# bingjeff/trex-gym

Hardware: AMD Instinct MI355X
Metric: env-steps/sec (whole node), trex.urdf 4096 envs per MI355X (higher is better)
Workload: dtype f32

## Files before the change

trex-gym_amd/csrc/device_model.h:

```cpp
#pragma once
#include <stdint.h>

#define TREX_TL 32
#define TREX_MAXD 6
#define TREX_MAXCH 4
#define TREX_CM_WORDS 320
#define TREX_MAXC 13

enum TrexParam {
  TP_DT, TP_SUBSTEPS, TP_ITERATIONS, TP_GRAVITY, TP_MOTOR_KP, TP_MOTOR_KD, TP_MOTOR_MAX_FORCE,
  TP_FLOOR_Z, TP_FRICTION, TP_ERP, TP_CONTACT_ERP, TP_CONTACT_MARGIN, TP_LINK_DAMPING,
  TP_MAX_COORD_VEL, TP_MAX_CONTACTS, TP_WARMSTART, TP_COUNT
};

struct TrexDeviceModel {
  int nb, maxdepth, head_body, nv;
  float prm[16];
  int n_substeps, n_iterations, max_contacts, pad0;
  float inv_dt, motor_max_impulse, pad1, pad2;
  float head_point[4];
  float base_pos0[4], base_quat0[4];
  int parent[TREX_TL], depth[TREX_TL];
  int obs_slot[TREX_TL];
  unsigned tree_pack[TREX_TL], child_pack[TREX_TL];
  int hull_range[TREX_TL][2];
  int pad4[64];
  int child[TREX_MAXCH][TREX_TL];
  unsigned desc_mask[TREX_TL];
  int hull_start[TREX_TL + 1];
  int cm_pack[TREX_TL];
  float axis[3][TREX_TL], jpos[3][TREX_TL], jrot[9][TREX_TL], com[3][TREX_TL], inertia[6][TREX_TL];
  float mass[TREX_TL], lower[TREX_TL], upper[TREX_TL], damp[TREX_TL], q_start[TREX_TL];
  float sphere[4][TREX_TL];
  float box_half[3][TREX_TL];
  int nchunk, pad3[3];
  int chunk_body[TREX_TL], chunk_v0[TREX_TL], chunk_v1[TREX_TL];
  float chunk_c[3][TREX_TL], chunk_h[3][TREX_TL];
  __attribute__((aligned(16))) int chunk_row[TREX_TL][4];
  float chunk_box[TREX_TL][8];
  int anc[TREX_MAXD][TREX_TL];
};
#define TREX_NO_DEPTH 255

#define TREX_BASE_FLAGS 13
#define TREX_BASE_IMPULSE 14
#define TREX_BASE_STEPS 15
#define TREX_MOTORS_BIT 256
#define TREX_BAL_PHASE 0
#define TREX_BAL_FINISHED 1
#define TREX_BAL_COUNTS 16
#define TREX_BAL_BINS 16
#define TREX_BAL_LISTS 48
#define TREX_BAL_WORDS(n) (TREX_BAL_LISTS + 2 * TREX_BAL_BINS * (size_t)(n))

struct TrexBatchArrays {
  float *base, *q, *qd, *mass_scale, *friction;
  int32_t domain;
  int32_t pad0_;
  int32_t *balance;
  int32_t max_episode_steps;
  int32_t pad_;
  float4 *hull;
  int num_links;
  const int *link_body;
  const float *link_tf;
  int num_visuals;
  const int *visual_body;
  const float *visual_tf;
};
#define TREX_WARM_WORDS 64
```

trex-gym_amd/csrc/host_tables.cpp:

```cpp
#include "host_tables.hpp"

#include "../../include/trex_policy.h"

#include <algorithm>
#include <array>
#include <cmath>
#include <cstdint>
#include <cstring>

namespace trex {

size_t row_block_bytes(size_t n, int stride, int width) { return ((n - 1) * (size_t)stride + (size_t)width) * sizeof(float); }

bool ranges_overlap(const void *a, size_t na, const void *b, size_t nb) {
  const uintptr_t p = (uintptr_t)a, q = (uintptr_t)b;
  return p < q + nb && q < p + na;
}

void check_env_offset(const std::string &who, uint32_t env_offset, int n_envs) {
  if ((uint64_t)env_offset + (uint64_t)n_envs > (1ull << 32)) throw Refusal(who + "env_offset + N is beyond 2^32");
}

size_t Layout::take(const char *name, size_t member_bytes, size_t align) {
  const size_t at = (bytes + align - 1) / align * align;
// ... 130 lines not shown
        const int g0 = h.hull_group_start[g], g1 = h.hull_group_start[g + 1];
        if (g1 <= g0) continue;
        int body = -1;
        for (int b = 0; b < h.nb; b++)
          if (h.hull_start[b] <= g0 && g1 <= h.hull_start[b + 1]) body = b;
        if (body < 0) ok = false;
        else units.push_back({body, g0, g1});
      }
    if (!ok || units.size() > TREX_TL) {
      units.clear();
      for (int b = 0; b < h.nb; b++)
        if (h.hull_start[b + 1] > h.hull_start[b]) units.push_back({b, h.hull_start[b], h.hull_start[b + 1]});
    }
    d.nchunk = (int)units.size();
    for (int k = 0; k < TREX_TL; k++) { d.chunk_body[k] = 0; d.chunk_v0[k] = 0; d.chunk_v1[k] = 0; }
    for (size_t k = 0; k < units.size(); k++) {
      const int v0 = units[k][1], v1 = units[k][2];
      trex::Vec3 lo{1e300, 1e300, 1e300}, hi{-1e300, -1e300, -1e300};
      for (int v = v0; v < v1; v++) {
        const trex::Vec3 &p = h.hull_xyz[v];
        const double r = h.hull_radius[v];
        lo = {std::min(lo.x, p.x - r), std::min(lo.y, p.y - r), std::min(lo.z, p.z - r)};
        hi = {std::max(hi.x, p.x + r), std::max(hi.y, p.y + r), std::max(hi.z, p.z + r)};
      }
      d.chunk_body[k] = units[k][0]; d.chunk_v0[k] = v0; d.chunk_v1[k] = v1;
      d.chunk_c[0][k] = (float)(0.5 * (lo.x + hi.x)); d.chunk_c[1][k] = (float)(0.5 * (lo.y + hi.y)); d.chunk_c[2][k] = (float)(0.5 * (lo.z + hi.z));
      d.chunk_h[0][k] = (float)(0.5 * (hi.x - lo.x) * (1 + 1e-6) + 1e-6); d.chunk_h[1][k] = (float)(0.5 * (hi.y - lo.y) * (1 + 1e-6) + 1e-6);
      d.chunk_h[2][k] = (float)(0.5 * (hi.z - lo.z) * (1 + 1e-6) + 1e-6);
    }
  }
  d.maxdepth = maxdepth;
  for (size_t k = 0; k < h.obs_order.size(); k++) d.obs_slot[h.obs_order[k]] = (int)k;
  for (int l = 0; l < TREX_TL; l++) {
    unsigned m = 0;
    if (l >= 1 && l < h.nb) {
      for (int b = 0; b < h.nb; b++)
        for (int i = b; i > 0; i = h.parent[i])
          if (i == l) { m |= 1u << b; break; }
    } else if (l >= h.nb && l < h.nb + 6) {
      m = (h.nb >= 32) ? 0xffffffffu : ((1u << h.nb) - 1u);
    }
    d.desc_mask[l] = m;
  }
  for (int l = 0; l < TREX_TL; l++) {
    const bool body = l < h.nb;
    const int parent = body ? d.parent[l] : 0, depth = body ? d.depth[l] : -1;
    d.tree_pack[l] = (unsigned)(parent < 0 ? 0 : parent) | (unsigned)(depth < 0 ? TREX_NO_DEPTH : depth) << 8;
    unsigned ch4 = 0u;
    for (int k = 0; k < TREX_MAXCH; k++) {
      const int c = body ? d.child[k][l] : -1;
      ch4 |= (unsigned)(c < 0 ? 255 : c) << (8 * k);
    }
    d.child_pack[l] = ch4;
    d.hull_range[l][0] = d.hull_start[body ? l : h.nb]; d.hull_range[l][1] = d.hull_start[body ? l + 1 : h.nb];
    const bool unit = l < d.nchunk;
    const int cb = d.chunk_body[l];
    d.chunk_row[l][0] = unit ? (cb | (d.cm_pack[cb] << 8)) : 0;
    d.chunk_row[l][1] = unit ? d.chunk_v0[l] : 0; d.chunk_row[l][2] = unit ? d.chunk_v1[l] : 0;
    d.chunk_row[l][3] = unit ? d.hull_start[cb] : 0;
    for (int c = 0; c < 3; c++) { d.chunk_box[l][c] = d.chunk_c[c][l]; d.chunk_box[l][4 + c] = d.chunk_h[c][l]; }
    d.chunk_box[l][3] = d.chunk_box[l][7] = 0.f;
  }
}

void tf12(const Tf &t, float out[12]) {
  for (int k = 0; k < 9; k++) out[k] = (float)t.R.m[k];
  out[9] = (float)t.t.x; out[10] = (float)t.t.y; out[11] = (float)t.t.z;
}

LinkPoint link_point(const Links &links, int link, const double x[3]) {
  const Tf &t = links.tf[link];
  const double tt[3] = {t.t.x, t.t.y, t.t.z};
  LinkPoint p;
  p.body = links.body[link];
  for (int r = 0; r < 3; r++)
    p.point[r] = (float)(t.R.m[3 * r] * x[0] + t.R.m[3 * r + 1] * x[1] + t.R.m[3 * r + 2] * x[2] + tt[r]);
  return p;
}

ProbeTable build_probe_table(const Links &links, const int32_t *link_host, const double *local_xyz_host, int num_probes) {
  ProbeTable t;
  t.body.resize((size_t)num_probes);
  t.tf.resize((size_t)num_probes * 12);
  for (int k = 0; k < num_probes; k++) {
    const int link = link_host[k];
    if (link < 0 || link >= (int)links.body.size())
      throw Refusal("trex_batch_set_link_probes: probe " + std::to_string(k) + ": link " + std::to_string(link) +
                    " out of range [0, " + std::to_string(links.body.size()) + ")");
    const double *x = local_xyz_host + 3 * (size_t)k;
    for (int c = 0; c < 3; c++)
      if (!std::isfinite(x[c]))
        throw Refusal("trex_batch_set_link_probes: probe " + std::to_string(k) + ": local_xyz is not finite");
    float *o = t.tf.data() + 12 * (size_t)k;
    tf12(links.tf[link], o);
    const LinkPoint p = link_point(links, link, x);
    t.body[k] = p.body;
    std::memcpy(o + 9, p.point, sizeof p.point);
  }
  return t;
}

ProxTable build_prox_table(int nb, const int32_t *body_host, const double *capsule_host, int num_capsules, const int32_t *pair_host,
                           int num_pairs) {
  const std::string me = "trex_batch_set_proximity_shapes: ";
  if (num_capsules < 0 || num_capsules > TREX_PROX_MAXCAPS)
    throw Refusal(me + "num_capsules " + std::to_string(num_capsules) + " outside [0, " + std::to_string(TREX_PROX_MAXCAPS) + "]");
// ... 993 lines not shown
```

trex-gym_amd/csrc/trex_step_body.h:

```cpp
#pragma once
#include <hip/hip_runtime.h>
#include <stdint.h>

#include <type_traits>
#include <utility>

#include "device_math.h"
#include "device_model.h"
#include "step_launch.h"

#define TL TREX_TL
#define MAXD TREX_MAXD
#define MAXCH TREX_MAXCH
#define MAXC TREX_MAXC

#ifndef TREX_STAMPS
#define TREX_STAMPS 0
#endif
#ifndef TREX_PAIR_MAX
#define TREX_PAIR_MAX 4096
#endif
#ifndef TREX_PAIR_LAUNCH
#define TREX_PAIR_LAUNCH (!TREX_STAMPS)
#endif
#ifndef TREX_ABLATE_EXACT_MATH
#define TREX_ABLATE_EXACT_MATH 0
#endif
#ifndef TREX_ABLATE_EXACT_QUAT
#define TREX_ABLATE_EXACT_QUAT 0
#endif
#ifndef TREX_ABLATE_PLAIN_COMMIT
#define TREX_ABLATE_PLAIN_COMMIT 0
#endif
#ifndef TREX_PRIO_MODE
#define TREX_PRIO_MODE 1
#endif
#if TREX_STAMPS
#define STAMP(i)                                                                          \
  do {                                                                                    \
    __builtin_amdgcn_sched_barrier(0);                                                    \
    const unsigned long long _t = __builtin_amdgcn_s_memtime();                           \
    __builtin_amdgcn_s_waitcnt(0xC07F);                                                   \
    if (args.debug && (threadIdx.x & 63) == 0) args.debug[4096 + (i) * args.n_envs + wg] += (float)(_t - stamp_last); \
    stamp_last = _t;                                                                      \
    __builtin_amdgcn_sched_barrier(0);                                                    \
  } while (0)
#define SUBSTAMP(i) STAMP(i)
#else
#define STAMP(i) asm volatile("; ---- phase mark " #i)
#define SUBSTAMP(i) do {} while (0)
#endif

namespace {

__device__ __forceinline__ float wshfl(float v, int src) { return __shfl(v, src, 64); }
__device__ __forceinline__ int wshfl(int v, int src) { return __shfl(v, src, 64); }
__device__ __forceinline__ float rl(float v, int src) { return __int_as_float(__builtin_amdgcn_readlane(__float_as_int(v), src)); }
__device__ __forceinline__ int rl(int v, int src) { return __builtin_amdgcn_readlane(v, src); }
__device__ __forceinline__ unsigned rl(unsigned v, int src) { return (unsigned)__builtin_amdgcn_readlane((int)v, src); }
__device__ __forceinline__ float uni(float v) { return __int_as_float(__builtin_amdgcn_readfirstlane(__float_as_int(v))); }
__device__ __forceinline__ int uni(int v) { return __builtin_amdgcn_readfirstlane(v); }
__device__ __forceinline__ float uni_sgpr(float v) {
  float r;
  asm volatile("s_nop 0\n\tv_readfirstlane_b32 %0, %1\n\ts_nop 1" : "=s"(r) : "v"(v));
  return r;
}
template <int CTRL>
__device__ __forceinline__ float dpp_mov(float v) {
  return __int_as_float(__builtin_amdgcn_update_dpp(0, __float_as_int(v), CTRL, 0xf, 0xf, true));
}
template <int CTRL>
__device__ __forceinline__ int dpp_mov_i(int v) {
  return __builtin_amdgcn_update_dpp(0, v, CTRL, 0xf, 0xf, true);
}
__device__ __forceinline__ float wsum(float v) {
  v += dpp_mov<0xB1>(v);
  v += dpp_mov<0x4E>(v);
  v += dpp_mov<0x141>(v);
  v += dpp_mov<0x140>(v);
  unsigned u = __float_as_uint(v);
  auto r = __builtin_amdgcn_permlane16_swap(u, u, false, false);
  v = __uint_as_float(r[0]) + __uint_as_float(r[1]);
  u = __float_as_uint(v);
  r = __builtin_amdgcn_permlane32_swap(u, u, false, false);
  return __uint_as_float(r[0]) + __uint_as_float(r[1]);
}
__device__ __forceinline__ float wminf(float v) {
  v = fminf(v, dpp_mov<0xB1>(v));
  v = fminf(v, dpp_mov<0x4E>(v));
  v = fminf(v, dpp_mov<0x141>(v));
  v = fminf(v, dpp_mov<0x140>(v));
  unsigned u = __float_as_uint(v);
  auto r = __builtin_amdgcn_permlane16_swap(u, u, false, false);
  v = fminf(__uint_as_float(r[0]), __uint_as_float(r[1]));
  u = __float_as_uint(v);
  r = __builtin_amdgcn_permlane32_swap(u, u, false, false);
  return fminf(__uint_as_float(r[0]), __uint_as_float(r[1]));
}
__device__ __forceinline__ int wmini(int v) {
  v = min(v, dpp_mov_i<0xB1>(v));
  v = min(v, dpp_mov_i<0x4E>(v));
  v = min(v, dpp_mov_i<0x141>(v));
  v = min(v, dpp_mov_i<0x140>(v));
  auto r = __builtin_amdgcn_permlane16_swap((unsigned)v, (unsigned)v, false, false);
  v = min((int)r[0], (int)r[1]);
  r = __builtin_amdgcn_permlane32_swap((unsigned)v, (unsigned)v, false, false);
  return min((int)r[0], (int)r[1]);
}
__device__ __forceinline__ float gmaxf(float v, int G) {
  v = fmaxf(v, dpp_mov<0xB1>(v));
  v = fmaxf(v, dpp_mov<0x4E>(v));
  v = fmaxf(v, dpp_mov<0x141>(v));
  if (G >= 16) v = fmaxf(v, dpp_mov<0x140>(v));
  if (G >= 32) {
    const unsigned u = __float_as_uint(v);
    const auto r = __builtin_amdgcn_permlane16_swap(u, u, false, false);
    v = fmaxf(__uint_as_float(r[0]), __uint_as_float(r[1]));
  }
  if (G >= 64) {
    const unsigned u = __float_as_uint(v);
    const auto r = __builtin_amdgcn_permlane32_swap(u, u, false, false);
    v = fmaxf(__uint_as_float(r[0]), __uint_as_float(r[1]));
  }
  return v;
}
__device__ __forceinline__ int gmini(int v, int G) {
  v = min(v, dpp_mov_i<0xB1>(v));
  v = min(v, dpp_mov_i<0x4E>(v));
  v = min(v, dpp_mov_i<0x141>(v));
  if (G >= 16) v = min(v, dpp_mov_i<0x140>(v));
  if (G >= 32) {
    const auto r = __builtin_amdgcn_permlane16_swap((unsigned)v, (unsigned)v, false, false);
    v = min((int)r[0], (int)r[1]);
  }
  if (G >= 64) {
    const auto r = __builtin_amdgcn_permlane32_swap((unsigned)v, (unsigned)v, false, false);
    v = min((int)r[0], (int)r[1]);
  }
// ... 51 lines not shown
  o1 = __builtin_fmaf(a[2], b[0], __builtin_fmaf(-a[0], b[2], o1));
  o2 = __builtin_fmaf(a[0], b[1], __builtin_fmaf(-a[1], b[0], o2));
}

struct Chol6 { float l[15], il[6]; };
__device__ __forceinline__ constexpr int lidx(int i, int j) { return i * (i - 1) / 2 + j; }
__device__ __forceinline__ float rsqrt_nr(float s) {
#if TREX_ABLATE_EXACT_MATH
  return 1.0f / sqrtf(s);
#endif
  const float r0 = __builtin_amdgcn_rsqf(s);
  const float e = __builtin_fmaf(-s * r0, r0, 1.0f);
  return __builtin_fmaf(0.5f * r0, e, r0);
}
__device__ __forceinline__ void chol6_factor(const float *a, Chol6 &c) {
#pragma unroll
  for (int j = 0; j < 6; j++) {
    float s = a[6 * j + j];
#pragma unroll
    for (int k = 0; k < j; k++) s -= c.l[lidx(j, k)] * c.l[lidx(j, k)];
    c.il[j] = rsqrt_nr(s);
#pragma unroll
    for (int i = j + 1; i < 6; i++) {
      float t = a[6 * i + j];
#pragma unroll
      for (int k = 0; k < j; k++) t -= c.l[lidx(i, k)] * c.l[lidx(j, k)];
      c.l[lidx(i, j)] = t * c.il[j];
    }
  }
}
__device__ __forceinline__ void chol6_solve(const Chol6 &c, const float *r, float *z) {
  float w[6];
#pragma unroll
  for (int i = 0; i < 6; i++) {
    float t = r[i];
#pragma unroll
    for (int k = 0; k < i; k++) t -= c.l[lidx(i, k)] * w[k];
    w[i] = t * c.il[i];
  }
#pragma unroll
  for (int i = 5; i >= 0; i--) {
    float t = w[i];
#pragma unroll
    for (int k = i + 1; k < 6; k++) t -= c.l[lidx(k, i)] * z[k];
    z[i] = t * c.il[i];
  }
}

constexpr int NJMAX = 25;
constexpr int NROW = NJMAX + 3 * MAXC;
static_assert(NROW == 64, "one constraint row per lane");
#define KROW_LANE(k) ((k) < 3 * MAXC - 1 ? NJMAX + 1 + (k) : 0)
constexpr int CLANE0 = NJMAX + 1;
__device__ __forceinline__ int warm_word(int l) {
  if (l >= 1 && l <= MAXC) return 4 * (l - 1);
  if (l == 0 || l >= CLANE0) { const int k = l == 0 ? 3 * MAXC - 1 : l - CLANE0; return 4 * (k / 3) + 1 + k % 3; }
  return -1;
}
constexpr int BREC = 5;
struct WaveLds {
  float4 body[32 * BREC];
  union {
    struct {
      float aba[32][28];
      float rtab[32][9];
    } t;
    float4 desc[64][4];
    float4 cg[160];
  } u;
  float cpt[MAXC][8];
  float st[6][TL];
  float xch[44];
};
enum { ST_Q, ST_QD, ST_TAU, ST_TARGET, ST_NQD, ST_MDG };
static_assert(sizeof(WaveLds) <= 10240, "16 envs per CU need <= 10 KB of LDS each");
constexpr int CG_WORDS = TREX_CM_WORDS;
struct CgLds {
  unsigned long long best[TL];
  float4 ent[TL][2];
  unsigned cm[CG_WORDS];
};
static_assert(sizeof(CgLds) <= sizeof(WaveLds::u), "contact-generation scratch fits the union area");

constexpr int ACT_GAINS = TREX_ACT_GAINS, ACT_ROWS = TREX_ACT_ROWS, SENS_ROWS = TREX_SENS_ROWS;

#ifndef TREX_GLOBAL
#define TREX_GLOBAL __attribute__((address_space(1)))
#endif
typedef const TREX_GLOBAL TrexDeviceModel *GlobalModel;
typedef int gm_int2 __attribute__((ext_vector_type(2)));
typedef int gm_int4 __attribute__((ext_vector_type(4)));
typedef float gm_float4 __attribute__((ext_vector_type(4)));
static_assert(offsetof(TrexDeviceModel, hull_range) % 8 == 0 && offsetof(TrexDeviceModel, chunk_row) % 16 == 0 &&
              offsetof(TrexDeviceModel, chunk_box) % 16 == 0, "the packed rows are fetched as aligned 8- and 16-byte words");

}

enum { FORM_SINGLE = TREX_KIND_STEP, FORM_MANY = TREX_KIND_STEP_MANY, FORM_RESET = TREX_KIND_RESET, FORM_DEBUG = TREX_KIND_STEP_DEBUG,
       FORM_PAIR, FORM_COUNT };
constexpr bool trex_step_variant_exists(int form, unsigned features) {
  const bool warm = features & TREX_FEAT_WARM, ext = features & TREX_FEAT_EXT, act = features & TREX_FEAT_ACT;
  if (TREX_STAMPS && ((features & ~TREX_FEAT_WARM) != 0u || form == FORM_DEBUG)) return false;
  if (form == FORM_PAIR && warm && act) return false;
  if (form == FORM_RESET && (ext || act)) return false;
  if (form == FORM_DEBUG && features != 0u) return false;
  return true;
}
#define WSYNC() do { if (PAIR) __builtin_amdgcn_fence(__ATOMIC_ACQ_REL, "wavefront"); else __syncthreads(); } while (0)
template <bool RESET, bool DEBUG, bool MULTI, bool PAIR = false, bool WARM = false, bool EXT = false, bool SENS = false, bool ACT = false>
__device__ __forceinline__ void trex_step_body(const TrexStepArgs &args, const int wg_in) {
  static_assert(!PAIR || (!RESET && !DEBUG && !MULTI), "the pair form exists for the product step launch only");
  static_assert(!(WARM && DEBUG), "the diagnostics dump has no warm-start form");
  static_assert(!EXT || (!RESET && !DEBUG), "the external wrench exists for the product step launches only");
  static_assert(!SENS || !DEBUG, "the diagnostics dump has no contact-sensor form");
  static_assert(!ACT || (!RESET && !DEBUG), "the actuator model exists for the product step launches only");
  __shared__ WaveLds Wpair[PAIR ? 2 : 1];
  __shared__ __attribute__((aligned(16))) unsigned char Gpair[PAIR ? sizeof(CgLds) : 16];
  const int wave = PAIR ? uni((int)threadIdx.x >> 6) : 0;
  int wave_v = PAIR ? (int)threadIdx.x >> 6 : 0;
  if (PAIR) asm volatile("" : "+v"(wave_v));
  WaveLds &W = Wpair[wave_v];
  __shared__ float4 Wrec[WARM ? (PAIR ? 2 : 1) : 1][MAXC];
  float4 *const Wr = Wrec[WARM ? wave_v : 0];
  const int wg = PAIR ? 2 * wg_in + wave : wg_in;
  const int tid = (int)threadIdx.x & 63;
  const TrexDeviceModel *__restrict__ M = args.model;
  constexpr bool EARLY = PAIR && (SENS || !(EXT || ACT));
  int nb_e = 0, maxdepth_e = 0, n_sub_e = 0, iters_e = 0, maxc_e = 0;
  float dt_e = 0.f, inv_dt_e = 0.f, mu_e = 0.f, floor_e = 0.f, margin_e = 0.f;
  if constexpr (EARLY) {
    nb_e = M->nb; maxdepth_e = M->maxdepth; n_sub_e = M->n_substeps; iters_e = M->n_iterations; maxc_e = M->max_contacts;
    const float dt_l = M->prm[TP_DT], inv_dt_l = M->inv_dt, mu_l = M->prm[TP_FRICTION];
    const float floor_l = M->prm[TP_FLOOR_Z], margin_l = M->prm[TP_CONTACT_MARGIN];
    dt_e = uni_sgpr(dt_l); inv_dt_e = uni_sgpr(inv_dt_l); mu_e = uni_sgpr(mu_l); floor_e = uni_sgpr(floor_l); margin_e = uni_sgpr(margin_l);
  }
  int env = wg;
  int bal_phase = 0;
  if (args.bal) {
    const int32_t *B = args.bal;
    bal_phase = uni(B[TREX_BAL_PHASE]);
    const int32_t *cnt = B + TREX_BAL_COUNTS + TREX_BAL_BINS * bal_phase;
    const int k = wg, q = k >> 10, m = min(1024, args.n_envs - (q << 10));
    int r = q == 0 ? k : (q << 10) + (m - 1 - (k & 1023));
    if (PAIR) {
      const int bq = wg_in >> 9, half = args.n_envs >> 1, bm = min(512, half - (bq << 9));
      const int pidx = bq == 0 ? wg_in : (bq << 9) + (bm - 1 - (wg_in & 511));
      r = wave == 0 ? pidx : args.n_envs - 1 - pidx;
    }
    const int lane_ = tid;
    const int mine = lane_ < TREX_BAL_BINS ? cnt[lane_] : 0;
    int b = TREX_BAL_BINS - 1, total = 0;
#pragma unroll
    for (int c = 0; c < TREX_BAL_BINS; c++) total += rl(mine, c);
    for (; b > 0; b--) {
      const int c = rl(mine, b);
      if (r < c) break;
      r -= c;
    }
    if (total == args.n_envs) {
      env = B[TREX_BAL_LISTS + (size_t)(bal_phase * TREX_BAL_BINS + b) * args.n_envs + r];
      if (env < 0 || env >= args.n_envs) env = wg;
    }
  }
  env = uni(env);

  const int nb = EARLY ? nb_e : M->nb, maxdepth = EARLY ? maxdepth_e : M->maxdepth;
  const float dt = EARLY ? dt_e : (PAIR ? uni_sgpr(M->prm[TP_DT]) : M->prm[TP_DT]);
  const float inv_dt = EARLY ? inv_dt_e : (PAIR ? uni_sgpr(M->inv_dt) : M->inv_dt);
  const float dt_half = PAIR ? uni_sgpr(0.5f * dt) : 0.5f * dt, dt2_quarter = PAIR ? uni_sgpr(0.25f * dt * dt) : 0.25f * dt * dt;
  const int nj = nb - 1;
  auto Mo = [&]() { const TrexDeviceModel *Mi = M; asm volatile("" : "+s"(Mi)); return (GlobalModel)Mi; };
  auto lane_id = [&]() {
    int l;
    asm volatile("v_mbcnt_lo_u32_b32 %0, -1, 0\n\tv_mbcnt_hi_u32_b32 %0, -1, %0" : "=v"(l));
    return l;
  };

  float pos[3], quat[4], bv[3], bw[3];
  const float mu = args.arr.domain ? uni(args.arr.friction[env]) : (EARLY ? mu_e : (PAIR ? uni_sgpr(M->prm[TP_FRICTION]) : M->prm[TP_FRICTION]));
  bool motors_on;
// ... 1047 lines not shown
      {
        float dxf[3];
        cross3(po, p + 3, dxf);
#pragma unroll
        for (int k = 0; k < 3; k++) p[k] += dxf[k];
      }
#pragma unroll
      for (int k = 0; k < 6; k++) r00[k] = live ? -p[k] : 0.f;
      chol6_solve(I0c, r00, z00);
      diag += dot6(r00, z00);
      inv0 = live ? 1.0f / diag : 0.f;
      GlobalModel Mi = Mo();
      const float cerp = Mi->prm[TP_CONTACT_ERP], erp = Mi->prm[TP_ERP], kp_m = Mi->prm[TP_MOTOR_KP], kd_m = Mi->prm[TP_MOTOR_KD];
      const float max_imp_m = Mi->motor_max_impulse, q_lo = Mi->lower[bl], q_hi = Mi->upper[bl];
      if (crow) {
        float tv = 0.f;
        if (cdir == 0) tv = (cdist > 0.f) ? -cdist * inv_dt : -cdist * cerp * inv_dt;
        float wxx[3];
        cross3(nw, cx, wxx);
        const float pv[3] = {nv[0] + wxx[0], nv[1] + wxx[1], nv[2] + wxx[2]};
        y = (tv - (jv + dot3(dir, pv))) * inv0;
      }
      if (mrow) {
        float kp = kp_m, kd = kd_m, max_imp = max_imp_m;
        const float q = W.st[ST_Q][bl], nqd = W.st[ST_NQD][bl];
        float target = W.st[ST_TARGET][bl], vt = 0.f;
        if constexpr (ACT) {
          const float *g = args.act + (size_t)env * (ACT_ROWS * TL) + bl;
          const int so = args.act_cols > nj ? 4 * TL : 0;
          kp = g[so]; kd = g[so + TL]; max_imp = g[2 * TL];
          const unsigned bit = 1u << bl;
          if (args.act_vel & bit) { vt = target; target = q; kp = 0.f; }
          else if (args.act_tor & bit) { target = q; kp = 0.f; kd = 0.f; max_imp = 0.f; }
        }
        W.st[ST_MDG][bl] = diag;
        if constexpr (ACT) {
          y = __builtin_fmaf(kd, vt - nqd, kp * (target - q) * inv_dt) * inv0;
        } else
        y = (kp * (target - q) * inv_dt + kd * (0.f - nqd)) * inv0;
        mhi = motors_on ? max_imp : 0.f;
        float pen = 0.f;
        if (q - q_lo <= 0.f) { pen = q - q_lo; ldir = 1.f; }
        else if (q_hi - q <= 0.f) { pen = q_hi - q; ldir = -1.f; }
        const float lim_rhs = (-pen * erp * inv_dt - ldir * nqd) * inv0;
        lr = lim_rhs - ldir * y;
      }
    }
    const unsigned lim_mask = (unsigned)__ballot(ldir != 0.f);
    WSYNC();
    {
      float *zs = reinterpret_cast<float *>(W.body);
#pragma unroll
      for (int k = 0; k < 6; k++) zs[64 * k + lt] = z00[k];
      float4 *dc = W.u.desc[lt];
      dc[0] = make_float4(__uint_as_float(ca0), zc0[0], zc0[1], zc0[2]);
      dc[1] = make_float4(zc0[3], zc0[4], zc0[5], z00[0]);
      dc[2] = make_float4(z00[1], z00[2], z00[3], z00[4]);
      dc[3] = make_float4(z00[5], 0.f, 0.f, 0.f);
      if (PAIR) {
        zs[64 * 6 + lt] = y; zs[64 * 7 + lt] = mhi; zs[64 * 8 + lt] = lr; zs[64 * 9 + lt] = ldir;
        asm volatile("" : "=v"(y), "=v"(mhi), "=v"(lr), "=v"(ldir));
      }
    }
    WSYNC();
    STAMP(5);
    RELANE();

    auto krow_lane = [](int k) { return k < 3 * MAXC - 1 ? CLANE0 + k : 0; };
    auto column = [&](int L, const float *m, float4 d0, float4 d1, float4 d2, float4 d3) {
      float a0_ = r00[0] * d1.w;
      a0_ = __builtin_fmaf(r00[1], d2.x, a0_); a0_ = __builtin_fmaf(r00[2], d2.y, a0_);
      a0_ = __builtin_fmaf(r00[3], d2.z, a0_); a0_ = __builtin_fmaf(r00[4], d2.w, a0_);
      a0_ = __builtin_fmaf(r00[5], d3.x, a0_);
      a0_ = __builtin_fmaf(m[0], d0.y, a0_); a0_ = __builtin_fmaf(m[1], d0.z, a0_); a0_ = __builtin_fmaf(m[2], d0.w, a0_);
      a0_ = __builtin_fmaf(m[3], d1.x, a0_); a0_ = __builtin_fmaf(m[4], d1.y, a0_); a0_ = __builtin_fmaf(m[5], d1.z, a0_);
      return -inv0 * a0_;
    };
    auto chain_mask = [&](float4 d0, float *m) {
      const unsigned lowdiff = (unsigned)__builtin_ctz((ca0 ^ __float_as_uint(d0.x)) | 0x40000000u);
#pragma unroll
      for (int d = 0; d < MAXD; d++) m[d] = (lowdiff >= 5u * (d + 1)) ? u0[d] : 0.f;
    };
    float Bm[NJMAX];
    {
      float4 n0 = W.u.desc[1][0], n1 = W.u.desc[1][1], n2 = W.u.desc[1][2], n3 = W.u.desc[1][3];
#pragma unroll
      for (int j = 1; j <= NJMAX; j++) {
        const float4 d0 = n0, d1 = n1, d2 = n2, d3 = n3;
        if (j < NJMAX) { n0 = W.u.desc[j + 1][0]; n1 = W.u.desc[j + 1][1]; n2 = W.u.desc[j + 1][2]; n3 = W.u.desc[j + 1][3]; }
        float m[MAXD];
        chain_mask(d0, m);
        Bm[j - 1] = column(j, m, d0, d1, d2, d3);
        asm volatile("" : "+v"(Bm[j - 1]));
        __builtin_amdgcn_sched_barrier(0);
      }
    }
    float Bc[3 * MAXC];
#pragma unroll
    for (int k = 0; k < 3 * MAXC; k++) asm volatile("" : "=v"(Bc[k]));
#pragma unroll
    for (int s = 0; s < MAXC; s++) {
      if (s >= s0) {
        float m[MAXD];
#pragma unroll
        for (int a = 0; a < 3; a++) {
          const float4 *dc = W.u.desc[krow_lane(3 * s + a)];
          const float4 d0 = dc[0], d1 = dc[1], d2 = dc[2], d3 = dc[3];
          if (a == 0) chain_mask(d0, m);
          Bc[3 * s + a] = column(0, m, d0, d1, d2, d3);
          asm volatile("" : "+v"(Bc[3 * s + a]));
        }
        __builtin_amdgcn_sched_barrier(0);
      }
    }
    STAMP(6);
    RELANE();

    if (PAIR) {
      const float *zs = reinterpret_cast<const float *>(W.body);
      y = zs[64 * 6 + lt]; mhi = zs[64 * 7 + lt]; lr = zs[64 * 8 + lt]; ldir = zs[64 * 9 + lt];
    }
    float lam = 0.f, lam_c = 0.f, lim_lam = 0.f;
    if (WARM) {
      const bool crow = lt == 0 || lt >= CLANE0;
      const int k = crow ? (lt == 0 ? 3 * MAXC - 1 : lt - CLANE0) : 0, slot = k / 3, dir = k - 3 * slot;
      const int key = (crow && slot >= s0) ? __float_as_int(W.cpt[slot - s0][5]) : 0;
      const float *rw = reinterpret_cast<const float *>(Wr);
      float l0 = 0.f;
#pragma unroll
      for (int r = 0; r < MAXC; r++)
        if (key != 0 && __float_as_int(rw[4 * r]) == key) l0 = rw[4 * r + 1 + dir];
      lam = Mo()->prm[TP_WARMSTART] * l0;
      const unsigned long long wm = __ballot(lam != 0.f);
      if (wm != 0ull) {
#pragma unroll
        for (int s = 0; s < MAXC; s++) {
          const unsigned long long sm = (1ull << KROW_LANE(3 * s)) | (1ull << KROW_LANE(3 * s + 1)) | (1ull << KROW_LANE(3 * s + 2));
          if (s >= s0 && (wm & sm) != 0ull) {
#pragma unroll
            for (int a = 0; a < 3; a++) y = __builtin_fmaf(Bc[3 * s + a], rl(lam, KROW_LANE(3 * s + a)), y);
          }
        }
      }
    }
    int dvec = 0;
    {
#define TREX_ROW(LANE, BCOL, LO, HI)                                                                   \
  {                                                                                                    \
    const float nl_ = __builtin_amdgcn_fmed3f(lam + y, (LO), (HI));                                    \
    const float d_ = nl_ - lam;                                                                        \
    const float sd_ = rl(d_, (LANE));                                                                  \
    if (vs == (LANE)) lam = nl_;                                                                       \
    y = __builtin_fmaf((BCOL), sd_, y);                                                                \
  }
#define TREX_POINT_ROWS(P)                                                                             \
                \
               "v_max_f32_e64 %[d], %[y], -%[lam]\n\t"                                                 \
               "v_add_f32_e32 %[t], %[lam], %[d]\n\t"                                                  \
               "v_readlane_b32 %[sd], %[d], %[ln" #P "]\n\t"                                           \
               "v_readlane_b32 %[snl], %[t], %[ln" #P "]\n\t"                                          \
               "s_nop 0\n\t"                                                                           \
               "v_fmac_f32_e32 %[y], %[sd], %[b0" #P "]\n\t"                                           \
               "v_mul_f32_e32 %[hi], %[snl], %[mu]\n\t"                                                \
                              \
               "v_sub_f32_e64 %[t], -%[hi], %[lam]\n\t"                                                \
// ... 357 lines not shown
                         TREX_JT_END(22)
                         "v_fmac_f32_e32 %[y], %[sd], %[b23]\n\t"
                         "s_branch 9f\n\t"
                         TREX_JT_END(23)
                         "v_fmac_f32_e32 %[y], %[sd], %[b24]\n\t"
                         "s_branch 9f\n\t"
                         TREX_JT_END(24)
                         "v_fmac_f32_e32 %[y], %[sd], %[b25]\n\t"
                         "9:\n\t"
                         ".if (9b - 8b) != 8 * 25 - 4\n\t.error \"limit-row jump table: entry 25 (no branch) does not end 8 * 25 - 4 bytes after entry 1\"\n\t.endif\n\t"
                         : [y] "+v"(y), [t] "=&s"(jt_)
                         : [sd] "s"(sd), [j] "s"(j), [b1] "v"(Bm[0]), [b2] "v"(Bm[1]), [b3] "v"(Bm[2]), [b4] "v"(Bm[3]), [b5] "v"(Bm[4]), [b6] "v"(Bm[5]), [b7] "v"(Bm[6]), [b8] "v"(Bm[7]), [b9] "v"(Bm[8]), [b10] "v"(Bm[9]), [b11] "v"(Bm[10]), [b12] "v"(Bm[11]), [b13] "v"(Bm[12]), [b14] "v"(Bm[13]), [b15] "v"(Bm[14]), [b16] "v"(Bm[15]), [b17] "v"(Bm[16]), [b18] "v"(Bm[17]), [b19] "v"(Bm[18]), [b20] "v"(Bm[19]), [b21] "v"(Bm[20]), [b22] "v"(Bm[21]), [b23] "v"(Bm[22]), [b24] "v"(Bm[23]), [b25] "v"(Bm[24])
                         : "vcc", "scc");
#undef TREX_JT_END
          }
        }
        TREX_MOTOR_SWEEP
        TREX_POINT_SWEEP(false, DEBUG)
      }
      }
#undef TREX_ROW
#undef TREX_MOTOR_SWEEP
#undef TREX_POINT_SWEEP
#undef TREX_STAMP_ALIVE
#undef TREX_POINTS_DISPATCH
#undef TREX_POINT_ROWS
#undef TREX_POINT_TEXT
#undef TREX_POINT_JUMP
#undef TREX_POINT_HEAD
#undef TREX_POINT_BLOCK
#undef TREX_POINT_BLOCK_END
#undef TREX_POINT_LAST
#undef TREX_POINTS3
#undef TREX_POINTS1
      lam -= lam_c;
    }
    if (WARM) {
      const int l = lane_id(), w = warm_word(l);
      const int slot = l >= 1 && l <= MAXC ? l - 1 : (l == 0 ? MAXC - 1 : (l - CLANE0) / 3);
      float v = 0.f;
      if (slot >= s0) v = (l >= 1 && l <= MAXC) ? W.cpt[slot - s0][5] : lam;
      if (w >= 0) reinterpret_cast<float *>(Wr)[w] = v;
    }
#if TREX_PRIO_MODE == 1
    prio_nc = nc;
    set_tree_priority(sub);
#endif
    STAMP(7);
    RELANE();
    REROW();

    const float lt0 = lam + (mlane ? ldir * lim_lam : 0.f);
    float dvj = 0.f;
#pragma unroll
    for (int j = 1; j <= NJMAX; j++) dvj -= Bm[j - 1] * rl(lt0, j);
#pragma unroll
    for (int s = 0; s < MAXC; s++) {
      if (s >= s0) {
#pragma unroll
        for (int a = 0; a < 3; a++) dvj -= Bc[3 * s + a] * rl(lam, krow_lane(3 * s + a));
      }
    }
    float dvb[6];
    {
      const float *zs = reinterpret_cast<const float *>(W.body);
#pragma unroll
      for (int k = 0; k < 6; k++) dvb[k] = uni(wsum(lt0 * zs[64 * k + lt]));
    }
    const float nimp = uni(wsum((!mlane && cdir == 0) ? lam : 0.f));
    const float mdg = W.st[ST_MDG][bl];
    const float dv = mrow ? dvj * mdg : 0.f;
    if constexpr (SENS) {
      const bool first = sub == 0 || sub == n_sub, last = sub + 1 >= n_sub;
      float *sw = args.sens + (size_t)env * (SENS_ROWS * TL) + bl;
      float acc[6] = {0.f, 0.f, 0.f, 0.f, 0.f, 0.f}, cb[3] = {0.f, 0.f, 0.f};
      if (is_body) {
#pragma unroll
        for (int k = 0; k < 3; k++) cb[k] = sw[(6 + k) * TL];
        if (!first) {
#pragma unroll
          for (int k = 0; k < 6; k++) acc[k] = sw[k * TL];
        }
      }
#pragma unroll
      for (int s = 0; s < MAXC; s++) {
        if (s >= s0) {
          const float fs[3] = {rl(lam, krow_lane(3 * s + 1)), rl(lam, krow_lane(3 * s + 2)), rl(lam, krow_lane(3 * s))};
          const float *cp = W.cpt[s - s0];
          if (__float_as_int(cp[0]) == lt) {
            const float d[3] = {cp[1] - cb[0], cp[2] - cb[1], cp[3] - cb[2]};
            float m[3];
            cross3(d, fs, m);
#pragma unroll
            for (int k = 0; k < 3; k++) { acc[k] += fs[k]; acc[3 + k] += m[k]; }
          }
        }
      }
      if (is_body) {
        const float scale = last ? inv_dt / (float)(sub == n_sub ? 1 : n_sub) : 1.f;
#pragma unroll
        for (int k = 0; k < 6; k++) sw[k * TL] = acc[k] * scale;
      }
    }

    if (DEBUG && args.debug && wg == 0) {
      float *D = args.debug;
      if (lt < TL) D[96 + lt] = dv;
      if (lt == 0) {
        for (int k = 0; k < 6; k++) D[96 + nb + k] = dvb[k];
        D[128] = (float)nc; D[129] = (float)lim_mask;
      }
      if (lt < TL) {
#pragma unroll
        for (int j = 1; j <= NJMAX; j++) D[160 + 32 * (j - 1) + lt] = mrow ? -Bm[j - 1] * mdg : 0.f;
      }
      for (int c = 0; c < nc; c++) {
        const float l0 = rl(lam, krow_lane(3 * (s0 + c))), l1 = rl(lam, krow_lane(3 * (s0 + c) + 1)), l2 = rl(lam, krow_lane(3 * (s0 + c) + 2));
        if (lt == 0) {
          float *C = D + 960 + c * 16;
          C[0] = (float)__float_as_int(W.cpt[c][0]); C[1] = W.cpt[c][1]; C[2] = W.cpt[c][2]; C[3] = W.cpt[c][3]; C[4] = W.cpt[c][4];
          C[11] = l0; C[12] = l1; C[13] = l2;
        }
// ... 164 lines not shown
```

Measured before the change: 12.20 million.

## Shrink constraint descriptors, hand-schedule dvj readlanes, interleave wave reductions

The per-row constraint descriptor in LDS shrinks from four float4s to three. The per-row chain key moves to a host-built chain_pack table, read through scalar constant loads for the motor columns and from a small LDS array for the contact slots. The dvj accumulation is written as inline asm that interleaves v_readlane with v_fmac, so readlane latency is hidden. The seven wave reductions (six body impulses plus the normal impulse) run as one batched DPP/permlane sequence instead of serially. Together these cut LDS traffic and dependency stalls in the solver's inner setup and update, at the cost of hard-coded asm tied to NJMAX==25 and MAXC==13 and a new model table.

```diff
diff --git a/trex-gym_amd/csrc/device_model.h b/trex-gym_amd/csrc/device_model.h
--- a/trex-gym_amd/csrc/device_model.h
+++ b/trex-gym_amd/csrc/device_model.h
@@ -24,7 +24,8 @@
   int obs_slot[TREX_TL];
   unsigned tree_pack[TREX_TL], child_pack[TREX_TL];
   int hull_range[TREX_TL][2];
-  int pad4[64];
+  unsigned chain_pack[TREX_TL];
+  int pad4[32];
   int child[TREX_MAXCH][TREX_TL];
   unsigned desc_mask[TREX_TL];
   int hull_start[TREX_TL + 1];
diff --git a/trex-gym_amd/csrc/host_tables.cpp b/trex-gym_amd/csrc/host_tables.cpp
--- a/trex-gym_amd/csrc/host_tables.cpp
+++ b/trex-gym_amd/csrc/host_tables.cpp
@@ -206,6 +206,10 @@
       ch4 |= (unsigned)(c < 0 ? 255 : c) << (8 * k);
     }
     d.child_pack[l] = ch4;
+    unsigned chain = 0u;
+    static_assert(5 * TREX_MAXD <= 32 && TREX_TL <= 32, "a chain packs into one word");
+    for (int b = body ? l : 0; b > 0 && d.depth[b] >= 1 && d.depth[b] <= TREX_MAXD; b = d.parent[b]) chain |= (unsigned)b << (5 * (d.depth[b] - 1));
+    d.chain_pack[l] = chain;
     d.hull_range[l][0] = d.hull_start[body ? l : h.nb]; d.hull_range[l][1] = d.hull_start[body ? l + 1 : h.nb];
     const bool unit = l < d.nchunk;
     const int cb = d.chunk_body[l];
diff --git a/trex-gym_amd/csrc/trex_step_body.h b/trex-gym_amd/csrc/trex_step_body.h
--- a/trex-gym_amd/csrc/trex_step_body.h
+++ b/trex-gym_amd/csrc/trex_step_body.h
@@ -35,6 +35,15 @@
 #ifndef TREX_PRIO_MODE
 #define TREX_PRIO_MODE 1
 #endif
+#ifndef TREX_DVJ_AHEAD
+#define TREX_DVJ_AHEAD 1
+#endif
+#ifndef TREX_WSUM_INTERLEAVE
+#define TREX_WSUM_INTERLEAVE 1
+#endif
+#ifndef TREX_DESC12
+#define TREX_DESC12 1
+#endif
 #if TREX_STAMPS
 #define STAMP(i)                                                                          \
   do {                                                                                    \
@@ -84,6 +93,32 @@
   u = __float_as_uint(v);
   r = __builtin_amdgcn_permlane32_swap(u, u, false, false);
   return __uint_as_float(r[0]) + __uint_as_float(r[1]);
+}
+template <int N>
+__device__ __forceinline__ void wsum_all(float (&v)[N]) {
+#define TREX_WSUM_DPP(CTRL)                                                                              \
+  _Pragma("unroll") for (int i = 0; i < N; i++) v[i] += dpp_mov<CTRL>(v[i]);                            \
+  __builtin_amdgcn_sched_barrier(0);
+  TREX_WSUM_DPP(0xB1)
+  TREX_WSUM_DPP(0x4E)
+  TREX_WSUM_DPP(0x141)
+  TREX_WSUM_DPP(0x140)
+#undef TREX_WSUM_DPP
+#define TREX_WSUM_SWAP(SWAP)                                                                             \
+  {                                                                                                      \
+    unsigned c[N];                                                                                       \
+    _Pragma("unroll") for (int i = 0; i < N; i++) asm volatile("v_mov_b32 %0, %1" : "=v"(c[i]) : "v"(v[i]));   \
+    _Pragma("unroll") for (int i = 0; i < N; i++) {                                                      \
+      const auto r = SWAP(__float_as_uint(v[i]), c[i], false, false);                                    \
+      v[i] = __uint_as_float(r[0]); c[i] = r[1];                                                         \
+    }                                                                                                    \
+    __builtin_amdgcn_sched_barrier(0);                                                                   \
+    _Pragma("unroll") for (int i = 0; i < N; i++) v[i] += __uint_as_float(c[i]);                         \
+    __builtin_amdgcn_sched_barrier(0);                                                                   \
+  }
+  TREX_WSUM_SWAP(__builtin_amdgcn_permlane16_swap)
+  TREX_WSUM_SWAP(__builtin_amdgcn_permlane32_swap)
+#undef TREX_WSUM_SWAP
 }
 __device__ __forceinline__ float wminf(float v) {
   v = fminf(v, dpp_mov<0xB1>(v));
@@ -241,6 +276,40 @@
 static_assert(NROW == 64, "one constraint row per lane");
 #define KROW_LANE(k) ((k) < 3 * MAXC - 1 ? NJMAX + 1 + (k) : 0)
 constexpr int CLANE0 = NJMAX + 1;
+#define TREX_DVJ_RL(T, LANE) "v_readlane_b32 %[" #T "], %[l], " #LANE "\n\t"
+#define TREX_DVJ_FM(T, B) "v_fmac_f32_e32 %[acc], %[" #T "], %[" #B "]\n\t"
+#define TREX_DVJ_FR(T, B, LANE) TREX_DVJ_FM(T, B) TREX_DVJ_RL(T, LANE)
+__device__ __forceinline__ void dvj_motor_columns(float &acc, float l, const float *B) {
+  static_assert(NJMAX == 25, "written out for the motor columns of lanes 1 .. 25");
+  int t0, t1;
+  asm volatile("s_nop 0\n\t"
+               TREX_DVJ_RL(t0, 1) TREX_DVJ_RL(t1, 2) "s_nop 0\n\t"
+               TREX_DVJ_FR(t0, b0, 3) TREX_DVJ_FR(t1, b1, 4) TREX_DVJ_FR(t0, b2, 5) TREX_DVJ_FR(t1, b3, 6)
+               TREX_DVJ_FR(t0, b4, 7) TREX_DVJ_FR(t1, b5, 8) TREX_DVJ_FR(t0, b6, 9) TREX_DVJ_FR(t1, b7, 10)
+               TREX_DVJ_FR(t0, b8, 11) TREX_DVJ_FR(t1, b9, 12) TREX_DVJ_FR(t0, b10, 13) TREX_DVJ_FR(t1, b11, 14)
+               TREX_DVJ_FR(t0, b12, 15) TREX_DVJ_FR(t1, b13, 16) TREX_DVJ_FR(t0, b14, 17) TREX_DVJ_FR(t1, b15, 18)
+               TREX_DVJ_FR(t0, b16, 19) TREX_DVJ_FR(t1, b17, 20) TREX_DVJ_FR(t0, b18, 21) TREX_DVJ_FR(t1, b19, 22)
+               TREX_DVJ_FR(t0, b20, 23) TREX_DVJ_FR(t1, b21, 24) TREX_DVJ_FR(t0, b22, 25)
+               TREX_DVJ_FM(t1, b23) "s_nop 0\n\t" TREX_DVJ_FM(t0, b24)
+               : [acc] "+v"(acc), [t0] "=&s"(t0), [t1] "=&s"(t1)
+               : [l] "v"(l), [b0] "v"(B[0]), [b1] "v"(B[1]), [b2] "v"(B[2]), [b3] "v"(B[3]), [b4] "v"(B[4]), [b5] "v"(B[5]), [b6] "v"(B[6]),
+                 [b7] "v"(B[7]), [b8] "v"(B[8]), [b9] "v"(B[9]), [b10] "v"(B[10]), [b11] "v"(B[11]), [b12] "v"(B[12]), [b13] "v"(B[13]),
+                 [b14] "v"(B[14]), [b15] "v"(B[15]), [b16] "v"(B[16]), [b17] "v"(B[17]), [b18] "v"(B[18]), [b19] "v"(B[19]),
+                 [b20] "v"(B[20]), [b21] "v"(B[21]), [b22] "v"(B[22]), [b23] "v"(B[23]), [b24] "v"(B[24]));
+}
+template <int S>
+__device__ __forceinline__ void dvj_point_columns(float &acc, float l, const float *B) {
+  int t0, t1;
+  asm volatile("s_nop 0\n\t"
+               "v_readlane_b32 %[t0], %[l], %[l0]\n\tv_readlane_b32 %[t1], %[l], %[l1]\n\ts_nop 0\n\t"
+               TREX_DVJ_FM(t0, b0) "v_readlane_b32 %[t0], %[l], %[l2]\n\t" TREX_DVJ_FM(t1, b1) "s_nop 0\n\t" TREX_DVJ_FM(t0, b2)
+               : [acc] "+v"(acc), [t0] "=&s"(t0), [t1] "=&s"(t1)
+               : [l] "v"(l), [b0] "v"(B[3 * S]), [b1] "v"(B[3 * S + 1]), [b2] "v"(B[3 * S + 2]),
+                 [l0] "n"(KROW_LANE(3 * S)), [l1] "n"(KROW_LANE(3 * S + 1)), [l2] "n"(KROW_LANE(3 * S + 2)));
+}
+#undef TREX_DVJ_FR
+#undef TREX_DVJ_FM
+#undef TREX_DVJ_RL
 __device__ __forceinline__ int warm_word(int l) {
   if (l >= 1 && l <= MAXC) return 4 * (l - 1);
   if (l == 0 || l >= CLANE0) { const int k = l == 0 ? 3 * MAXC - 1 : l - CLANE0; return 4 * (k / 3) + 1 + k % 3; }
@@ -255,6 +324,10 @@
       float rtab[32][9];
     } t;
     float4 desc[64][4];
+    struct {
+      float4 desc[64][3];
+      unsigned pchain[16];
+    } d12;
     float4 cg[160];
   } u;
   float cpt[MAXC][8];
@@ -277,6 +350,7 @@
 #define TREX_GLOBAL __attribute__((address_space(1)))
 #endif
 typedef const TREX_GLOBAL TrexDeviceModel *GlobalModel;
+typedef const __attribute__((address_space(4))) TrexDeviceModel *ConstModel;
 typedef int gm_int2 __attribute__((ext_vector_type(2)));
 typedef int gm_int4 __attribute__((ext_vector_type(4)));
 typedef float gm_float4 __attribute__((ext_vector_type(4)));
@@ -315,6 +389,9 @@
   const int tid = (int)threadIdx.x & 63;
   const TrexDeviceModel *__restrict__ M = args.model;
   constexpr bool EARLY = PAIR && (SENS || !(EXT || ACT));
+  constexpr bool DVJ_AHEAD = TREX_DVJ_AHEAD && PAIR && !SENS;
+  constexpr bool WSUM_INTERLEAVE = TREX_WSUM_INTERLEAVE && !(PAIR && SENS && ACT);
+  constexpr bool DESC12 = TREX_DESC12 && !WARM;
   int nb_e = 0, maxdepth_e = 0, n_sub_e = 0, iters_e = 0, maxc_e = 0;
   float dt_e = 0.f, inv_dt_e = 0.f, mu_e = 0.f, floor_e = 0.f, margin_e = 0.f;
   if constexpr (EARLY) {
@@ -1468,11 +1545,19 @@
       float *zs = reinterpret_cast<float *>(W.body);
 #pragma unroll
       for (int k = 0; k < 6; k++) zs[64 * k + lt] = z00[k];
-      float4 *dc = W.u.desc[lt];
-      dc[0] = make_float4(__uint_as_float(ca0), zc0[0], zc0[1], zc0[2]);
-      dc[1] = make_float4(zc0[3], zc0[4], zc0[5], z00[0]);
-      dc[2] = make_float4(z00[1], z00[2], z00[3], z00[4]);
-      dc[3] = make_float4(z00[5], 0.f, 0.f, 0.f);
+      if constexpr (DESC12) {
+        float4 *dc = W.u.d12.desc[lt];
+        dc[0] = make_float4(zc0[0], zc0[1], zc0[2], zc0[3]);
+        dc[1] = make_float4(zc0[4], zc0[5], z00[0], z00[1]);
+        dc[2] = make_float4(z00[2], z00[3], z00[4], z00[5]);
+        if (lt >= CLANE0 && cdir == 0) W.u.d12.pchain[(lt - CLANE0) / 3] = ca0;
+      } else {
+        float4 *dc = W.u.desc[lt];
+        dc[0] = make_float4(__uint_as_float(ca0), zc0[0], zc0[1], zc0[2]);
+        dc[1] = make_float4(zc0[3], zc0[4], zc0[5], z00[0]);
+        dc[2] = make_float4(z00[1], z00[2], z00[3], z00[4]);
+        dc[3] = make_float4(z00[5], 0.f, 0.f, 0.f);
+      }
       if (PAIR) {
         zs[64 * 6 + lt] = y; zs[64 * 7 + lt] = mhi; zs[64 * 8 + lt] = lr; zs[64 * 9 + lt] = ldir;
         asm volatile("" : "=v"(y), "=v"(mhi), "=v"(lr), "=v"(ldir));
@@ -1483,50 +1568,103 @@
     RELANE();
 
     auto krow_lane = [](int k) { return k < 3 * MAXC - 1 ? CLANE0 + k : 0; };
-    auto column = [&](int L, const float *m, float4 d0, float4 d1, float4 d2, float4 d3) {
-      float a0_ = r00[0] * d1.w;
-      a0_ = __builtin_fmaf(r00[1], d2.x, a0_); a0_ = __builtin_fmaf(r00[2], d2.y, a0_);
-      a0_ = __builtin_fmaf(r00[3], d2.z, a0_); a0_ = __builtin_fmaf(r00[4], d2.w, a0_);
-      a0_ = __builtin_fmaf(r00[5], d3.x, a0_);
-      a0_ = __builtin_fmaf(m[0], d0.y, a0_); a0_ = __builtin_fmaf(m[1], d0.z, a0_); a0_ = __builtin_fmaf(m[2], d0.w, a0_);
-      a0_ = __builtin_fmaf(m[3], d1.x, a0_); a0_ = __builtin_fmaf(m[4], d1.y, a0_); a0_ = __builtin_fmaf(m[5], d1.z, a0_);
-      return -inv0 * a0_;
-    };
-    auto chain_mask = [&](float4 d0, float *m) {
-      const unsigned lowdiff = (unsigned)__builtin_ctz((ca0 ^ __float_as_uint(d0.x)) | 0x40000000u);
-#pragma unroll
-      for (int d = 0; d < MAXD; d++) m[d] = (lowdiff >= 5u * (d + 1)) ? u0[d] : 0.f;
-    };
-    float Bm[NJMAX];
-    {
-      float4 n0 = W.u.desc[1][0], n1 = W.u.desc[1][1], n2 = W.u.desc[1][2], n3 = W.u.desc[1][3];
-#pragma unroll
-      for (int j = 1; j <= NJMAX; j++) {
-        const float4 d0 = n0, d1 = n1, d2 = n2, d3 = n3;
-        if (j < NJMAX) { n0 = W.u.desc[j + 1][0]; n1 = W.u.desc[j + 1][1]; n2 = W.u.desc[j + 1][2]; n3 = W.u.desc[j + 1][3]; }
-        float m[MAXD];
-        chain_mask(d0, m);
-        Bm[j - 1] = column(j, m, d0, d1, d2, d3);
-        asm volatile("" : "+v"(Bm[j - 1]));
-        __builtin_amdgcn_sched_barrier(0);
-      }
-    }
-    float Bc[3 * MAXC];
-#pragma unroll
-    for (int k = 0; k < 3 * MAXC; k++) asm volatile("" : "=v"(Bc[k]));
-#pragma unroll
-    for (int s = 0; s < MAXC; s++) {
-      if (s >= s0) {
-        float m[MAXD];
-#pragma unroll
-        for (int a = 0; a < 3; a++) {
-          const float4 *dc = W.u.desc[krow_lane(3 * s + a)];
-          const float4 d0 = dc[0], d1 = dc[1], d2 = dc[2], d3 = dc[3];
-          if (a == 0) chain_mask(d0, m);
-          Bc[3 * s + a] = column(0, m, d0, d1, d2, d3);
-          asm volatile("" : "+v"(Bc[3 * s + a]));
-        }
-        __builtin_amdgcn_sched_barrier(0);
+    float Bm[NJMAX], Bc[3 * MAXC];
+    if constexpr (DESC12) {
+      auto column = [&](const float *m, float4 d0, float4 d1, float4 d2) {
+        float a0_ = r00[0] * d1.z;
+        a0_ = __builtin_fmaf(r00[1], d1.w, a0_); a0_ = __builtin_fmaf(r00[2], d2.x, a0_);
+        a0_ = __builtin_fmaf(r00[3], d2.y, a0_); a0_ = __builtin_fmaf(r00[4], d2.z, a0_);
+        a0_ = __builtin_fmaf(r00[5], d2.w, a0_);
+        a0_ = __builtin_fmaf(m[0], d0.x, a0_); a0_ = __builtin_fmaf(m[1], d0.y, a0_); a0_ = __builtin_fmaf(m[2], d0.z, a0_);
+        a0_ = __builtin_fmaf(m[3], d0.w, a0_); a0_ = __builtin_fmaf(m[4], d1.x, a0_); a0_ = __builtin_fmaf(m[5], d1.y, a0_);
+        return -inv0 * a0_;
+      };
+      auto chain_mask = [&](unsigned chain, float *m) {
+        const unsigned lowdiff = (unsigned)__builtin_ctz((ca0 ^ chain) | 0x40000000u);
+#pragma unroll
+        for (int d = 0; d < MAXD; d++) m[d] = (lowdiff >= 5u * (d + 1)) ? u0[d] : 0.f;
+      };
+      {
+        const TrexDeviceModel *Mp = M;
+        asm volatile("" : "+s"(Mp));
+        const ConstModel Mc = (ConstModel)Mp;
+        typedef const __attribute__((address_space(4))) gm_int4 *ChainRow;
+        gm_int4 cw = *(ChainRow)&Mc->chain_pack[0];
+        const float4 (*D)[3] = W.u.d12.desc;
+        float4 n0 = D[1][0], n1 = D[1][1], n2 = D[1][2];
+#pragma unroll
+        for (int j = 1; j <= NJMAX; j++) {
+          const float4 d0 = n0, d1 = n1, d2 = n2;
+          if (j < NJMAX) { n0 = D[j + 1][0]; n1 = D[j + 1][1]; n2 = D[j + 1][2]; }
+          if (j % 4 == 0) cw = *(ChainRow)&Mc->chain_pack[j];
+          float m[MAXD];
+          chain_mask((unsigned)cw[j % 4], m);
+          Bm[j - 1] = column(m, d0, d1, d2);
+          asm volatile("" : "+v"(Bm[j - 1]));
+          __builtin_amdgcn_sched_barrier(0);
+        }
+      }
+#pragma unroll
+      for (int k = 0; k < 3 * MAXC; k++) asm volatile("" : "=v"(Bc[k]));
+#pragma unroll
+      for (int s = 0; s < MAXC; s++) {
+        if (s >= s0) {
+          float m[MAXD];
+          chain_mask(W.u.d12.pchain[s], m);
+#pragma unroll
+          for (int a = 0; a < 3; a++) {
+            const float4 *dc = W.u.d12.desc[krow_lane(3 * s + a)];
+            const float4 d0 = dc[0], d1 = dc[1], d2 = dc[2];
+            Bc[3 * s + a] = column(m, d0, d1, d2);
+            asm volatile("" : "+v"(Bc[3 * s + a]));
+          }
+          __builtin_amdgcn_sched_barrier(0);
+        }
+      }
+    } else {
+      auto column = [&](int L, const float *m, float4 d0, float4 d1, float4 d2, float4 d3) {
+        float a0_ = r00[0] * d1.w;
+        a0_ = __builtin_fmaf(r00[1], d2.x, a0_); a0_ = __builtin_fmaf(r00[2], d2.y, a0_);
+        a0_ = __builtin_fmaf(r00[3], d2.z, a0_); a0_ = __builtin_fmaf(r00[4], d2.w, a0_);
+        a0_ = __builtin_fmaf(r00[5], d3.x, a0_);
+        a0_ = __builtin_fmaf(m[0], d0.y, a0_); a0_ = __builtin_fmaf(m[1], d0.z, a0_); a0_ = __builtin_fmaf(m[2], d0.w, a0_);
+        a0_ = __builtin_fmaf(m[3], d1.x, a0_); a0_ = __builtin_fmaf(m[4], d1.y, a0_); a0_ = __builtin_fmaf(m[5], d1.z, a0_);
+        return -inv0 * a0_;
+      };
+      auto chain_mask = [&](float4 d0, float *m) {
+        const unsigned lowdiff = (unsigned)__builtin_ctz((ca0 ^ __float_as_uint(d0.x)) | 0x40000000u);
+#pragma unroll
+        for (int d = 0; d < MAXD; d++) m[d] = (lowdiff >= 5u * (d + 1)) ? u0[d] : 0.f;
+      };
+      {
+        float4 n0 = W.u.desc[1][0], n1 = W.u.desc[1][1], n2 = W.u.desc[1][2], n3 = W.u.desc[1][3];
+#pragma unroll
+        for (int j = 1; j <= NJMAX; j++) {
+          const float4 d0 = n0, d1 = n1, d2 = n2, d3 = n3;
+          if (j < NJMAX) { n0 = W.u.desc[j + 1][0]; n1 = W.u.desc[j + 1][1]; n2 = W.u.desc[j + 1][2]; n3 = W.u.desc[j + 1][3]; }
+          float m[MAXD];
+          chain_mask(d0, m);
+          Bm[j - 1] = column(j, m, d0, d1, d2, d3);
+          asm volatile("" : "+v"(Bm[j - 1]));
+          __builtin_amdgcn_sched_barrier(0);
+        }
+      }
+#pragma unroll
+      for (int k = 0; k < 3 * MAXC; k++) asm volatile("" : "=v"(Bc[k]));
+#pragma unroll
+      for (int s = 0; s < MAXC; s++) {
+        if (s >= s0) {
+          float m[MAXD];
+#pragma unroll
+          for (int a = 0; a < 3; a++) {
+            const float4 *dc = W.u.desc[krow_lane(3 * s + a)];
+            const float4 d0 = dc[0], d1 = dc[1], d2 = dc[2], d3 = dc[3];
+            if (a == 0) chain_mask(d0, m);
+            Bc[3 * s + a] = column(0, m, d0, d1, d2, d3);
+            asm volatile("" : "+v"(Bc[3 * s + a]));
+          }
+          __builtin_amdgcn_sched_barrier(0);
+        }
       }
     }
     STAMP(6);
@@ -1990,22 +2128,43 @@
 
     const float lt0 = lam + (mlane ? ldir * lim_lam : 0.f);
     float dvj = 0.f;
-#pragma unroll
-    for (int j = 1; j <= NJMAX; j++) dvj -= Bm[j - 1] * rl(lt0, j);
-#pragma unroll
-    for (int s = 0; s < MAXC; s++) {
-      if (s >= s0) {
-#pragma unroll
-        for (int a = 0; a < 3; a++) dvj -= Bc[3 * s + a] * rl(lam, krow_lane(3 * s + a));
-      }
-    }
-    float dvb[6];
-    {
+    if constexpr (DVJ_AHEAD) {
+      float acc = 0.f;
+      dvj_motor_columns(acc, lt0, Bm);
+      static_assert(MAXC == 13, "the point slots are written out");
+#define TREX_DVJ_SLOT(S) if (S >= s0) dvj_point_columns<S>(acc, lam, Bc);
+      TREX_DVJ_SLOT(0) TREX_DVJ_SLOT(1) TREX_DVJ_SLOT(2) TREX_DVJ_SLOT(3) TREX_DVJ_SLOT(4) TREX_DVJ_SLOT(5) TREX_DVJ_SLOT(6)
+      TREX_DVJ_SLOT(7) TREX_DVJ_SLOT(8) TREX_DVJ_SLOT(9) TREX_DVJ_SLOT(10) TREX_DVJ_SLOT(11) TREX_DVJ_SLOT(12)
+#undef TREX_DVJ_SLOT
+      dvj = 0.f - acc;
+    } else {
+#pragma unroll
+      for (int j = 1; j <= NJMAX; j++) dvj -= Bm[j - 1] * rl(lt0, j);
+#pragma unroll
+      for (int s = 0; s < MAXC; s++) {
+        if (s >= s0) {
+#pragma unroll
+          for (int a = 0; a < 3; a++) dvj -= Bc[3 * s + a] * rl(lam, krow_lane(3 * s + a));
+        }
+      }
+    }
+    float dvb[6], nimp;
+    if constexpr (WSUM_INTERLEAVE) {
       const float *zs = reinterpret_cast<const float *>(W.body);
+      float red[7];
+#pragma unroll
+      for (int k = 0; k < 6; k++) red[k] = lt0 * zs[64 * k + lt];
+      red[6] = (!mlane && cdir == 0) ? lam : 0.f;
+      wsum_all(red);
+#pragma unroll
+      for (int k = 0; k < 6; k++) dvb[k] = uni(red[k]);
+      nimp = uni(red[6]);
+    } else {
+      const float *zs = reinterpret_cast<const float *>(W.body);
 #pragma unroll
       for (int k = 0; k < 6; k++) dvb[k] = uni(wsum(lt0 * zs[64 * k + lt]));
-    }
-    const float nimp = uni(wsum((!mlane && cdir == 0) ? lam : 0.f));
+      nimp = uni(wsum((!mlane && cdir == 0) ? lam : 0.f));
+    }
     const float mdg = W.st[ST_MDG][bl];
     const float dv = mrow ? dvj * mdg : 0.f;
     if constexpr (SENS) {
```

Result: no change. 12.24 million (median of 6 runs) (+0.4%).
